# kevalmorabia97/CoVA-Web-Object-Detection

Hardware: AMD Instinct MI355X
Metric: webpages/sec fwd+bwd (90 bboxes, K=24) (higher is better)
Workload: dtype f32

## Files before the change

### cova-web-object-detection_amd/csrc/conv_wino4.hip

```cpp
#include "common.h"
#include "mma.h"
#include "bn_tail.h"
#include "options.h"
#include <type_traits>

#ifndef W4_ABL
#define W4_ABL 0
#endif

#ifdef W4_TRACE
__device__ unsigned long long g_w4_trace[2 * 20 * 8];
#define W4_STAMP(row, slot)                                                                                  \
    do {                                                                                                     \
        const int r__ = (row);                                                                               \
        if (blockIdx.x == 0 && (wave == 0 || wave == 4) && r__ >= 0 && r__ < 20 && lane == 0)                \
            g_w4_trace[((wave >> 2) * 20 + r__) * 8 + (slot)] = __builtin_amdgcn_s_memtime();                \
    } while (0)
#else
#define W4_STAMP(row, slot) do { } while (0)
#endif

namespace {

namespace w4 {
constexpr int TH = 8, TW = 32, PH = TH + 2, PW = TW + 2, NPIX = PH * PW;
constexpr int THREADS = 512;
constexpr int SLOT_FLOATS = NPIX * 16;
constexpr int TMP_CI = 16 * 36 + 4;
constexpr int TMP_FLOATS = 8 * TMP_CI;
constexpr int VROW = 36;
constexpr int V_FLOATS = 8 * 16 * VROW;
constexpr int U_FLOATS = 8 * 8 * 9 * 64 * 4;
constexpr int U_SPLIT_DWORDS = 2 * 8 * 18 * 3 * 256;
constexpr int U_TOTAL = U_FLOATS + 2 * U_SPLIT_DWORDS;
}

// ... 4 lines not shown
    o[0] = fmaf(4.f, d[0], fmaf(-5.f, d[2], d[4]));
    o[1] = a + b;
    o[2] = a - b;
    o[3] = c + e;
    o[4] = c - e;
    o[5] = fmaf(4.f, d[1], fmaf(-5.f, d[3], d[5]));
}

__device__ __forceinline__ void at6(const float (&m)[6], float (&o)[4])
{
    const float s1 = m[1] + m[2], d1 = m[1] - m[2], s2 = m[3] + m[4], d2 = m[3] - m[4];
    o[0] = m[0] + s1 + s2;
    o[1] = fmaf(2.f, d2, d1);
    o[2] = fmaf(4.f, s2, s1);
    o[3] = fmaf(8.f, d2, d1) + m[5];
}

struct W4Epi {
    const float *addend, *act, *z, *mean, *invstd, *msc, *msh;
    const uint32_t *act_bits;
    int inf_relu;
    int inference;
};

struct W4Args {
    const float *in, *in2, *u;
    float *out, *stat_part;
    int H, W, tiles_x, tiles_y, ntiles;
    const float *pro_abc;
    int pro_relu;
    W4Epi epi;
    BnTail tail;
};

__device__ __attribute__((aligned(256))) float g_w4_zero_page[64];

__device__ __forceinline__ float quad_class_sum(float v)
{
    v += __builtin_bit_cast(float, __builtin_amdgcn_update_dpp(0, __builtin_bit_cast(int, v), 0x124, 0xF, 0xF, true));
    v += __builtin_bit_cast(float, __builtin_amdgcn_update_dpp(0, __builtin_bit_cast(int, v), 0x128, 0xF, 0xF, true));
    v += __shfl_xor(v, 16, 64);
    v += __shfl_xor(v, 32, 64);
    return v;
}

template <bool STATS, int PRO, bool ADD, int BN>
__global__ __launch_bounds__(w4::THREADS, 1) void conv3x3_c64_wino4_kernel(const W4Args a)
{
    using namespace w4;
    typedef const W4Args __attribute__((address_space(4))) *KArgs;
    auto late_args = [&]() -> KArgs {
        unsigned long long kp = (unsigned long long)__builtin_amdgcn_kernarg_segment_ptr();
        asm volatile("" : "+s"(kp));
        return (KArgs)kp;
    };
    constexpr int NSLOT = 2;
    constexpr int NT = PRO == 2 ? 2 : 1;
    constexpr int IN_FLOATS = NSLOT * SLOT_FLOATS;
    __shared__ __attribute__((aligned(16))) float lds[NT * IN_FLOATS + 2 * TMP_FLOATS + 2 * V_FLOATS];
    __shared__ __attribute__((aligned(16))) float s_epi[BN ? 256 : 4];
    __shared__ float s_pro[PRO ? 192 : 1];
    __shared__ __attribute__((aligned(16))) float s_red[STATS ? 8 * 32 : 4];
    float *s_in = lds;
    float *s_in2 = lds + IN_FLOATS;
    float *s_tmp1 = lds + NT * IN_FLOATS;
    float *s_tmp0 = s_tmp1 + TMP_FLOATS;
// ... 271 lines not shown
        mfma_range(8, 12);
        item_finish(1, it, s2);
        item_read(2, it, slot2, coff2, tmp_w, tmp_r, v_w);
        mfma_range(12, 16);
        read_v(1);
        item_finish(2, it, s2);
        mfma_range(16, 36);
        } else {
        Item it0, it1, it2;
        item_read(0, it0, slot2, coff2, tmp_w, tmp_r, v_w);
        item_read(1, it1, slot2, coff2, tmp_w, tmp_r, v_w);
        item_read(2, it2, slot2, coff2, tmp_w, tmp_r, v_w);
        read_v(0);
        W4_STAMP(g - 32, 1);
        mfma_range(0, 16);
        W4_STAMP(g - 32, 2);
        read_v(1);
        mfma_range(16, 18);
        item_finish(0, it0, s2);
        item_finish(1, it1, s2);
        item_finish(2, it2, s2);
        W4_STAMP(g - 32, 3);
        mfma_range(18, 36);
        }
        W4_STAMP(g - 32, 4);
        wait_planes(g);
        W4_STAMP(g - 32, 5);
        lds_barrier();
        W4_STAMP(g - 32, 6);
    };

    constexpr bool W4_SIGNED_TILES = false;
    constexpr bool w4_neg = false;
#include "conv_wino4_epi.h"

#pragma unroll 1
    for (int g = 0; g < G; g += 2) {
        iteration(g, std::integral_constant<int, 0>{}, Ea);
        iteration(g + 1, std::integral_constant<int, 1>{}, Ea);
        if ((g & 7) == 6) tile_epilogue(g >> 3);
    }
#include "conv_wino4_tail.h"
}

struct PrepW { const float *w[4]; };
__device__ void prep_wino4s_element(const float *__restrict__ w, uint16_t *__restrict__ u_fwd, uint16_t *__restrict__ u_dgrad, int idx);
__global__ void prep_wino4_kernel(const PrepW pw, float *__restrict__ u_fwd, float *__restrict__ u_dgrad)
{
    const int idx = blockIdx.x * blockDim.x + threadIdx.x;
    if (idx >= w4::U_FLOATS) return;
    const float *__restrict__ w = pw.w[blockIdx.y];
    u_fwd += (size_t)blockIdx.y * w4::U_TOTAL;
    u_dgrad += (size_t)blockIdx.y * w4::U_TOTAL;
    const int e = idx & 3, lane = (idx >> 2) & 63, rest = idx >> 8;
    const int q = rest % 9, ws = rest / 9, wv = ws & 7, s = ws >> 3;
    const int n = 4 * q + e, kg = n / 18, p = n - 18 * kg;
    const int cog = wv & 3, ph = wv >> 2, kq = lane >> 4, l15 = lane & 15;
    const int o = cog * 16 + l15, c = 8 * s + 4 * kg + kq;
    const int il = p / 6, j = p % 6;
    const int i = ph == 0 ? il : (il == 0 ? 5 : 2 + il);
    const float G[6][3] = {{0.25f, 0.f, 0.f},
                           {-1.f / 6, -1.f / 6, -1.f / 6},
                           {-1.f / 6, 1.f / 6, -1.f / 6},
                           {1.f / 24, 1.f / 12, 1.f / 6},
                           {1.f / 24, -1.f / 12, 1.f / 6},
                           {0.f, 0.f, 1.f}};
    double uf = 0.0, ud = 0.0;
#pragma unroll
    for (int r = 0; r < 3; ++r)
#pragma unroll
        for (int t = 0; t < 3; ++t) {
            const double coef = (double)G[i][r] * (double)G[j][t];
            uf += coef * (double)w[((o * 64 + c) * 3 + r) * 3 + t];
// ... 5 lines not shown
}

#include "conv_wino4_split.h"

}

#ifdef W4_TRACE
COVA_API int cova_w4_trace_read(unsigned long long *host)
{
    return (int)hipMemcpyFromSymbol(host, HIP_SYMBOL(g_w4_trace), sizeof(unsigned long long) * 320);
}
#endif

COVA_API int cova_conv3x3_wino4_num_tiles(int B, int H, int W)
{
    return B * cdiv(W, w4::TW) * cdiv(H, w4::TH);
}

static int w4_grid(int B, int H, int W)
{
    const int tiles_x = cdiv(W, w4::TW), tiles_y = cdiv(H, w4::TH);
    int g = cova_internal_persistent_grid2(B * tiles_x * tiles_y, 1);
    const int len_odd = B * tiles_x * (tiles_y / 2);
    if (len_odd > 0) {
        if (g > 2 * len_odd) g = 2 * len_odd;
        g &= ~1;
        if (g < 2) g = 2;
    }
    return g;
}

COVA_API int cova_conv3x3_wino4_num_partials(int B, int H, int W) { return w4_grid(B, H, W); }

COVA_API int cova_conv3x3_wino4_u_floats(void) { return w4::U_TOTAL; }

COVA_API int cova_conv3x3_wino4_prep_multi(const float *w0, const float *w1, const float *w2, const float *w3,
                                           float *u_fwd, float *u_dgrad, void *stream)
{
    COVA_REQUIRE(w0 && u_fwd && u_dgrad);
    const PrepW pw{{w0, w1, w2, w3}};
    const int n = w1 == nullptr ? 1 : w2 == nullptr ? 2 : w3 == nullptr ? 3 : 4;
    hipLaunchKernelGGL(prep_wino4_kernel, dim3(cdiv(w4::U_FLOATS, 256), n), dim3(256), 0, (hipStream_t)stream, pw, u_fwd,
                       u_dgrad);
    COVA_LAUNCH_CHECK();
    return COVA_OK;
}

COVA_API int cova_conv3x3_wino4_prep(const float *w_oihw, float *u_fwd, float *u_dgrad, void *stream)
{
    return cova_conv3x3_wino4_prep_multi(w_oihw, nullptr, nullptr, nullptr, u_fwd, u_dgrad, stream);
}

namespace {

template <bool STATS, int PRO, bool ADD, int BN>
void launch_w4(const W4Args &a, int grid, hipStream_t st)
{
    if constexpr (PRO != 2) {
        if (!cova_options().wino4_f32) {
            W4Args b = a;
            b.u = a.u + w4::U_FLOATS;
            hipLaunchKernelGGL((conv3x3_c64_wino4s_kernel<STATS, PRO, ADD, BN>), dim3(grid), dim3(w4::THREADS), 0, st, b);
            return;
        }
    }
    hipLaunchKernelGGL((conv3x3_c64_wino4_kernel<STATS, PRO, ADD, BN>), dim3(grid), dim3(w4::THREADS), 0, st, a);
// ... 93 lines not shown
```

### cova-web-object-detection_amd/csrc/conv_wino4_epi.h

```cpp
    float *xw = s_x + (cog * 8 * 64 + lane) * 4;
    auto tile_epilogue = [&](int k) {
        int ph_e = ph;
        asm volatile("" : "+s"(ph_e));
        const float cf_s = ph_e == 0 ? 1.f : 4.f, cf_t0 = ph_e == 0 ? 1.f : 0.f;
        const float cf_d = ph_e == 0 ? 1.f : 8.f, cf_t1 = ph_e == 0 ? 0.f : 1.f, cf_h = ph_e == 0 ? 1.f : 2.f;
        if (W4_ABL & 32) {
#pragma unroll
            for (int p = 0; p < 18; ++p) { asm volatile("" ::"v"(acc[p])); acc[p] = f32x4{0.f, 0.f, 0.f, 0.f}; }
            return;
        }
        const int tile_ = tile_of(k);
        const int tx = tile_ % a.tiles_x, ty = (tile_ / a.tiles_x) % a.tiles_y, b = tile_ / (a.tiles_x * a.tiles_y);
        const float tsign = (W4_SIGNED_TILES && w4_neg) ? -1.f : 1.f;
        const KArgs la = late_args();
        const float *e_addend = la->epi.addend, *e_z = la->epi.z, *e_act = la->epi.act;
        float *e_out = la->out;
        float yo[2][4][4], ys[2][4][4];
#pragma unroll
        for (int r = 0; r < 4; ++r) {
            float tm[3][4];
#pragma unroll
            for (int il = 0; il < 3; ++il) {
                float m[6], o[4];
#pragma unroll
                for (int j = 0; j < 6; ++j) m[j] = acc[il * 6 + j][r];
                at6(m, o);
#pragma unroll
                for (int j = 0; j < 4; ++j) tm[il][j] = o[j];
            }
#pragma unroll
            for (int j = 0; j < 4; ++j) {
                const float sm = tm[1][j] + tm[2][j], df = tm[1][j] - tm[2][j];
                yo[0][j][r] = fmaf(cf_s, sm, cf_t0 * tm[0][j]);
                yo[1][j][r] = fmaf(cf_d, df, cf_t1 * tm[0][j]);
                ys[0][j][r] = sm;
                ys[1][j][r] = cf_h * df;
            }
        }
        const int t2 = lane >> 2, cq = cog * 16 + (lane & 3) * 4;
        const int oy0 = ty * TH + 4 * (t2 >> 3) + 2 * ph, ox0 = tx * TW + 4 * (t2 & 7);
        const size_t img = (size_t)b * H * W * 64;
        struct Ops { float4 ad[4], z4[4], a4[4]; };
        const bool bits = BN == 2 && la->epi.act_bits != nullptr;
        auto offs = [&](int io, int j) {
            return (unsigned)((min(oy0 + io, H - 1) * W + min(ox0 + j, W - 1)) * 64 + cq);
        };
        auto load_ops = [&](int io, Ops &o) {
#pragma unroll
            for (int j = 0; j < 4; ++j) {
                const unsigned off = offs(io, j);
                o.ad[j] = o.z4[j] = o.a4[j] = make_float4(0.f, 0.f, 0.f, 0.f);
                if (ADD) o.ad[j] = *reinterpret_cast<const float4 *>(e_addend + img + off);
                if (BN == 1 || BN == 2) o.z4[j] = *reinterpret_cast<const float4 *>(e_z + img + off);
                if (BN == 2) {
                    if (bits) {
                        const uint32_t wd = la->epi.act_bits[((size_t)b * H * W * 64 + off) >> 5] >> (cq & 31);
                        o.a4[j] = make_float4((float)(wd & 1u), (float)((wd >> 1) & 1u), (float)((wd >> 2) & 1u),
                                              (float)((wd >> 3) & 1u));
                    } else {
                        o.a4[j] = *reinterpret_cast<const float4 *>(e_act + img + off);
                    }
                }
            }
        };
        Ops ops;
        W4_STAMP(16 + 2 * (k - 4), 0);
        if (ADD || BN) load_ops(0, ops);
        float4 rx[2][4];
        auto put = [&]() {
#pragma unroll
            for (int io = 0; io < 2; ++io)
#pragma unroll
                for (int j = 0; j < 4; ++j)
                    *reinterpret_cast<float4 *>(xw + (io * 4 + j) * 256) = make_float4(ys[io][j][0], ys[io][j][1], ys[io][j][2], ys[io][j][3]);
        };
        auto get = [&]() {
#pragma unroll
            for (int io = 0; io < 2; ++io)
#pragma unroll
                for (int j = 0; j < 4; ++j) rx[io][j] = *reinterpret_cast<const float4 *>(xw + (io * 4 + j) * 256);
        };
        W4_STAMP(16 + 2 * (k - 4), 1);
        if (ph == 1) put();
        if (!(W4_ABL & 512)) lds_barrier();
        if (ph == 0) { get(); put(); }
        if (!(W4_ABL & 512)) lds_barrier();
        if (ph == 1) get();
        if (!(W4_ABL & 512)) lds_barrier();
        W4_STAMP(16 + 2 * (k - 4), 2);
// ... 8 lines not shown
        float ssum[4] = {0.f, 0.f, 0.f, 0.f}, ssq[4] = {0.f, 0.f, 0.f, 0.f};
#pragma unroll
        for (int io = 0; io < 2; ++io) {
            const int oy = oy0 + io;
            float mu[4] = {0.f, 0.f, 0.f, 0.f}, is[4] = {0.f, 0.f, 0.f, 0.f}, msc[4] = {0.f, 0.f, 0.f, 0.f}, msh[4] = {0.f, 0.f, 0.f, 0.f};
            if (BN) {
                const float4 m4 = *reinterpret_cast<const float4 *>(s_epi + cq), i4 = *reinterpret_cast<const float4 *>(s_epi + 64 + cq);
                mu[0] = m4.x; mu[1] = m4.y; mu[2] = m4.z; mu[3] = m4.w;
                is[0] = i4.x; is[1] = i4.y; is[2] = i4.z; is[3] = i4.w;
                if (BN == 1 || BN == 3) {
                    const float4 s4 = *reinterpret_cast<const float4 *>(s_epi + 128 + cq), h4 = *reinterpret_cast<const float4 *>(s_epi + 192 + cq);
                    msc[0] = s4.x; msc[1] = s4.y; msc[2] = s4.z; msc[3] = s4.w;
                    msh[0] = h4.x; msh[1] = h4.y; msh[2] = h4.z; msh[3] = h4.w;
                }
            }
#pragma unroll
            for (int j = 0; j < 4; ++j) {
                const bool ok = oy < H && ox0 + j < W;
                const int src = ((lane & 3) * 16 + (lane >> 2)) * 4;
                float own[4];
#pragma unroll
                for (int r = 0; r < 4; ++r)
                    own[r] = __builtin_bit_cast(float, __builtin_amdgcn_ds_bpermute(src, __builtin_bit_cast(int, yo[io][j][r])));
                const float adv[4] = {ops.ad[j].x, ops.ad[j].y, ops.ad[j].z, ops.ad[j].w};
                const float zv[4] = {ops.z4[j].x, ops.z4[j].y, ops.z4[j].z, ops.z4[j].w};
                const float av[4] = {ops.a4[j].x, ops.a4[j].y, ops.a4[j].z, ops.a4[j].w};
                float o[4];
#pragma unroll
                for (int r = 0; r < 4; ++r) {
                    float v = W4_SIGNED_TILES ? own[r] * tsign : own[r];
                    if (BN == 3) {
                        v = fmaf(msc[r], v, msh[r]);
                        if (ADD) v += adv[r];
                        if (la->epi.inf_relu) v = v > 0.f ? v : 0.f;
                        o[r] = v;
                        continue;
                    }
                    if (ADD) v += adv[r];
                    if (BN) {
                        const float gate = BN == 2 ? av[r] : fmaf(msc[r], zv[r], msh[r]);
                        if (!(gate > 0.f) || !ok) v = 0.f;
                        ssum[r] += v;
                        ssq[r] += v * ((zv[r] - mu[r]) * is[r]);
                    } else if (STATS) {
                        if (!ok) v = 0.f;
                        ssum[r] += v;
                        ssq[r] += v * v;
                    }
                    o[r] = v;
                }
                if (!(W4_ABL & 256) && ok)
                    *reinterpret_cast<float4 *>(e_out + img + (unsigned)(((oy0 + io) * W + ox0 + j) * 64 + cq)) =
                        make_float4(o[0], o[1], o[2], o[3]);
            }
            if ((ADD || BN) && io == 0) {
                __builtin_amdgcn_sched_barrier(0);
                load_ops(1, ops);
            }
        }
        W4_STAMP(16 + 2 * (k - 4), 3);
        if (STATS) {
#pragma unroll
            for (int r = 0; r < 4; ++r) {
                ssum[r] = quad_class_sum(ssum[r]);
                ssq[r] = quad_class_sum(ssq[r]);
            }
            if (lane < 4) {
// ... 13 lines not shown
```

### cova-web-object-detection_amd/csrc/conv_wino4_split.h

```cpp
namespace w4s {
constexpr int SLOT_BYTES = w4::NPIX * 64 + 64;
constexpr int PLANES_BYTES = 4 * SLOT_BYTES;
constexpr int VBLK = 1024;
constexpr int VBUF_BYTES = 12 * 3 * VBLK;
constexpr int LDS_BYTES = PLANES_BYTES + 2 * VBUF_BYTES;
constexpr int U_KSTEP_BYTES = 8 * 18 * 3 * 1024;
constexpr int U_DWORDS = 2 * U_KSTEP_BYTES / 4;
}

#ifndef W4S_ABL
#define W4S_ABL 0
#endif
#ifndef W4S_LEAD
#define W4S_LEAD 3
#endif

__device__ __forceinline__ f32x4 mfma16bf(u32x4 a, u32x4 b, f32x4 c)
{
    return __builtin_amdgcn_mfma_f32_16x16x32_bf16(__builtin_bit_cast(bf16x8, a), __builtin_bit_cast(bf16x8, b), c, 0, 0, 0);
}

template <bool STATS, int PRO, bool ADD, int BN>
__global__ __launch_bounds__(w4::THREADS, 1) void conv3x3_c64_wino4s_kernel(const W4Args a)
{
    using namespace w4;
    static_assert(PRO != 2, "the two-tensor prologue runs on the f32 main loop");
    typedef const W4Args __attribute__((address_space(4))) *KArgs;
    auto late_args = [&]() -> KArgs {
        unsigned long long kp = (unsigned long long)__builtin_amdgcn_kernarg_segment_ptr();
        asm volatile("" : "+s"(kp));
        return (KArgs)kp;
    };
    __shared__ __attribute__((aligned(256))) float lds[w4s::LDS_BYTES / 4];
    __shared__ __attribute__((aligned(16))) float s_epi[BN ? 256 : 4];
    __shared__ __attribute__((aligned(16))) float s_pro[PRO ? 192 : 4];
    __shared__ __attribute__((aligned(16))) float s_red[STATS ? 8 * 32 : 4];
    char *const s_planes = reinterpret_cast<char *>(lds);
    char *const s_vb = s_planes + w4s::PLANES_BYTES;
    float *s_x = reinterpret_cast<float *>(s_vb + w4s::VBUF_BYTES);
    const int tid = threadIdx.x, lane = tid & 63;
    const int wave = __builtin_amdgcn_readfirstlane(tid >> 6);
    const int cog = wave & 3, ph = wave >> 2;
    const int l15 = lane & 15, kq = lane >> 4;
    const int H = a.H, W = a.W;
    if (PRO && tid < 192) s_pro[tid] = late_args()->pro_abc[tid];
    if (BN && tid >= 256) {
        const int c = tid & 63, kind = (tid >> 6) & 3;
        const KArgs la = late_args();
        const float *src = kind == 0 ? la->epi.mean : kind == 1 ? la->epi.invstd : kind == 2 ? la->epi.msc : la->epi.msh;
        const bool used = BN == 3 ? kind >= 2 : (kind < 2 || BN == 1);
        s_epi[kind * 64 + c] = used ? src[c] : 0.f;
    }
    if (PRO || BN) __syncthreads();

    const int Gd = (int)gridDim.x;
    const bool lists = a.tiles_y > 1;
    const int w4_par = lists ? (int)(blockIdx.x & 1) : 0;
    const int Gp = lists ? Gd >> 1 : Gd;
    int bp = lists ? (int)(blockIdx.x >> 1) : (int)blockIdx.x;
    if ((Gd & 7) == 0) bp = lists ? (int)((blockIdx.x & 7) >> 1) * (Gd >> 3) + (int)(blockIdx.x >> 3)
                                  : (int)(blockIdx.x & 7) * (Gd >> 3) + (int)(blockIdx.x >> 3);
    const int nrow = lists ? (w4_par ? a.tiles_y >> 1 : (a.tiles_y + 1) >> 1) : a.tiles_y;
    const int per_page = nrow * a.tiles_x;
    const int lenp = (a.ntiles / (a.tiles_x * a.tiles_y)) * per_page;
    const int nk = bp < lenp ? (lenp - bp + Gp - 1) / Gp : 0;
    auto tile_of = [&](int k) {
        const int m = bp + (k < nk ? k : nk - 1) * Gp;
        const int b_ = m / per_page, rem = m - b_ * per_page, j = rem / a.tiles_x, tx_ = rem - j * a.tiles_x;
        return (b_ * a.tiles_y + (lists ? 2 * j + w4_par : j)) * a.tiles_x + tx_;
    };
    const bool w4_neg = w4_par != 0;

    const unsigned pl_base = (unsigned)(size_t)(lds_void *)s_planes;
    const float *tbase = a.in;
    unsigned rel16[3] = {0, 0, 0};
    bool in16[3] = {false, false, false};
    const int q16 = lane & 3;
    auto px16 = [&](int i) { return 16 * (wave + 8 * i) + (lane >> 2); };
#pragma unroll
    for (int i = 0; i < 3; ++i) {
        const int px = px16(i), r = px / PW, c = px - r * PW;
        rel16[i] = (unsigned)((r * W + c) * 64 + 4 * q16) * 4u;
    }
    auto plane_src = [&](int k) {
        const int tile_ = tile_of(k);
        const int tx = tile_ % a.tiles_x, ty = (tile_ / a.tiles_x) % a.tiles_y, b = tile_ / (a.tiles_x * a.tiles_y);
        const long long org = ((long long)b * H * W + (long long)(ty * TH - 1) * W + (tx * TW - 1)) * 64;
        tbase = a.in + org;
#pragma unroll
        for (int i = 0; i < 3; ++i) {
            int px = px16(i);
            asm volatile("" : "+v"(px));
            const int r = (px * 241) >> 13, c = px - r * PW;
            const int gy = ty * TH + r - 1, gx = tx * TW + c - 1;
            in16[i] = gy >= 0 && gy < H && gx >= 0 && gx < W;
        }
    };
    auto copy_piece = [&](const int gi, const int slot, const int i) {
        if (W4S_ABL & 8) return;
        const int j = wave + 8 * i;
        if (j < 22 && px16(i) < NPIX) {
            const unsigned dst = pl_base + (unsigned)slot * w4s::SLOT_BYTES + j * 1024;
            if (in16[i]) copy16_to_lds(tbase + 16 * gi, rel16[i], dst);
            else copy16_to_lds(g_w4_zero_page, (unsigned)q16 * 16u, dst);
        }
    };

    const int hf = wave & 1;
    const int tt = 4 * (wave >> 1) + (lane >> 4), cp = lane & 15;
    const int tt_rd = (W4S_ABL & 512) ? (tt & ~1) : tt;
    const char *rd = s_planes + (cp >> 3) * w4s::SLOT_BYTES + ((4 * (tt_rd >> 3) + hf) * PW + 4 * (tt_rd & 7)) * 64 + (cp & 7) * 8;
    char *vw = s_vb + hf * (6 * 3 * w4s::VBLK) + tt * 64 + ((((cp >> 2) ^ ((4 - (tt >> 2)) & 3))) << 4) + (cp & 3) * 4;
    const char *vr = s_vb + ph * (6 * 3 * w4s::VBLK) + l15 * 64 + ((kq ^ ((4 - (l15 >> 2)) & 3)) << 4);
    unsigned m30 = 0x3FFFFFFFu;
    bool edge = false;
    auto masks = [&](int k) {
        const int tile_ = tile_of(k);
        const int tx_ = tile_ % a.tiles_x, ty_ = (tile_ / a.tiles_x) % a.tiles_y;
        edge = ty_ == 0 || ty_ * TH + TH + 1 > H || tx_ == 0 || tx_ * TW + TW + 1 > W;
        const int gy0 = ty_ * TH + 4 * (tt >> 3) + hf - 1, gx0 = tx_ * TW + 4 * (tt & 7) - 1;
        unsigned cm = 0, m = 0;
#pragma unroll
        for (int c = 0; c < 6; ++c) cm |= (gx0 + c >= 0 && gx0 + c < W) ? (1u << c) : 0u;
#pragma unroll
        for (int r = 0; r < 5; ++r) m |= (gy0 + r >= 0 && gy0 + r < H) ? (cm << (6 * r)) : 0u;
        m30 = m;
    };

    float T[3][6][2];
#pragma unroll
    for (int i = 0; i < 3; ++i)
#pragma unroll
        for (int c = 0; c < 6; ++c) T[i][c][0] = T[i][c][1] = 0.f;
    auto column = [&](const int c, const int par, const int ks, auto edge_t) {
        constexpr bool EDGE = decltype(edge_t)::value;
        if (W4S_ABL & 1) return;
        const char *p = rd + par * (2 * w4s::SLOT_BYTES) + c * 64;
        float x[5][2];
#pragma unroll
        for (int r = 0; r < 5; ++r) {
            const float2 v = *reinterpret_cast<const float2 *>(p + r * (PW * 64));
            x[r][0] = v.x; x[r][1] = v.y;
        }
        if (PRO) {
            const float2 A2 = *reinterpret_cast<const float2 *>(s_pro + 32 * ks + 2 * cp);
            const float2 C2 = *reinterpret_cast<const float2 *>(s_pro + 128 + 32 * ks + 2 * cp);
            const float Av[2] = {A2.x, A2.y}, Cv[2] = {C2.x, C2.y};
#pragma unroll
            for (int r = 0; r < 5; ++r)
#pragma unroll
                for (int e = 0; e < 2; ++e) {
// ... 12 lines not shown
                o1 = u + v; o2 = u - v;
            } else {
                const float u = x[3][e] - x[1][e], v = 2.f * (x[2][e] - x[0][e]);
                o1 = u + v; o2 = u - v;
            }
            T[0][c][e] = o0; T[1][c][e] = o1; T[2][c][e] = o2;
        }
    };
    auto column_e = [&](const int c, const int par, const int ks) {
        if (PRO && edge) column(c, par, ks, std::true_type{});
        else column(c, par, ks, std::false_type{});
    };
    auto row_stage = [&](const int sn, float (&o)[6][2]) {
        if (W4S_ABL & 1) return;
#pragma unroll
        for (int e = 0; e < 2; ++e) {
            const float d[6] = {T[sn][0][e], T[sn][1][e], T[sn][2][e], T[sn][3][e], T[sn][4][e], T[sn][5][e]};
            float r[6];
            bt6(d, r);
#pragma unroll
            for (int j = 0; j < 6; ++j) o[j][e] = r[j];
        }
    };
    auto split_write = [&](const int j, const int parw, const float (&o)[6][2]) {
        if (W4S_ABL & 1) return;
        uint32_t q0, q1, q2;
        bf3_split_pair(o[j][0], o[j][1], q0, q1, q2);
        char *d = vw + parw * w4s::VBUF_BYTES + j * (3 * w4s::VBLK);
        *reinterpret_cast<uint32_t *>(d) = q0;
        *reinterpret_cast<uint32_t *>(d + w4s::VBLK) = q1;
        *reinterpret_cast<uint32_t *>(d + 2 * w4s::VBLK) = q2;
    };

    const char *const ubase = reinterpret_cast<const char *>(a.u) + (size_t)wave * (18 * 3 * 1024) +
                              (w4_neg ? (size_t)w4::U_SPLIT_DWORDS * 4 : (size_t)0);
    const unsigned ulane = (unsigned)lane * 16u;
    constexpr int UR = W4S_LEAD + 1;
    static_assert(36 % UR == 0, "ring size must divide the 36-position stream");
    u32x4 Ub[UR][3];
    auto load_u = [&](const int n_, const int slot) {
        if (W4S_ABL & 16) return;
        const int n = n_ % 36;
        const char *ub_t = ubase;
        const int ks = (W4S_ABL & 128) ? 0 : n / 18, p = (W4S_ABL & 128) ? 0 : n - 18 * ks;
        if (W4S_ABL & 256) {
#pragma unroll
            for (int q = 0; q < 3; ++q) Ub[slot][q] = *reinterpret_cast<const u32x4 *>(vr + ((n % 12) * 3 + q) * w4s::VBLK);
            return;
        }
        const char *bp = ub_t + (size_t)ks * w4s::U_KSTEP_BYTES + p * 3072;
        unsigned ul = ulane;
        asm volatile("" : "+v"(ul));
#pragma unroll
        for (int q = 0; q < 3; ++q) Ub[slot][q] = *reinterpret_cast<const u32x4 *>(bp + q * 1024 + ul);
    };

    plane_src(0);
#pragma unroll
    for (int i = 0; i < 3; ++i)
#pragma unroll
        for (int g = 0; g < 4; ++g) copy_piece(g, g, i);
#pragma unroll
    for (int n = 0; n < UR; ++n)
#pragma unroll
        for (int q = 0; q < 3; ++q) Ub[n][q] = u32x4{0u, 0u, 0u, 0u};
#pragma unroll
    for (int n = 0; n < W4S_LEAD; ++n) load_u(n, n);
    __builtin_amdgcn_s_waitcnt(0);
    __syncthreads();
    if (PRO) masks(0);
    {
#pragma unroll
        for (int c = 0; c < 6; ++c) column_e(c, 0, 0);
        float o[6][2];
        row_stage(0, o);
#pragma unroll
        for (int j = 0; j < 6; ++j) split_write(j, 0, o);
    }
    if (STATS && tid < 256) s_red[tid] = 0.f;
    __syncthreads();

    f32x4 acc[18];
#pragma unroll
    for (int p = 0; p < 18; ++p) acc[p] = f32x4{0.f, 0.f, 0.f, 0.f};

    auto step = [&](const int k, auto ks_t, auto s_t) {
        constexpr int KS = decltype(ks_t)::value, S = decltype(s_t)::value;
        constexpr int TI = 3 * KS + S, PAR = TI & 1, NPAR = (KS + 1) & 1, NKS = NPAR;
        if (KS == 0 && S == 0) plane_src(k + 1);
        copy_piece(2 * KS, 2 * KS, S);
        copy_piece(2 * KS + 1, 2 * KS + 1, S);
        if (PRO && KS == 1 && S == 1) masks(k + 1);
        const char *vp = vr + PAR * w4s::VBUF_BYTES;
        u32x4 Vr[2][3];
        auto read_v = [&](const int j, const int b) {
            if (W4S_ABL & 64) return;
#pragma unroll
            for (int q = 0; q < 3; ++q) Vr[b][q] = *reinterpret_cast<const u32x4 *>(vp + (j * 3 + q) * w4s::VBLK);
        };
        float o[6][2];
        if (W4S_ABL & 64) {
#pragma unroll
            for (int q = 0; q < 3; ++q) Vr[0][q] = Vr[1][q] = u32x4{0u, 0u, 0u, 0u};
        }
        read_v(0, 0);
        if (S != 2) row_stage(S + 1, o);
#pragma unroll
        for (int j = 0; j < 6; ++j) {
            constexpr int n0 = TI * 6;
            const int n = n0 + j, ub = n % UR;
            if (j < 5) read_v(j + 1, (j + 1) & 1);
            if (!(W4S_ABL & 4)) {
                f32x4 c = acc[S * 6 + j];
                const u32x4 *U = Ub[ub], *V = Vr[j & 1];
                c = mfma16bf(U[2], V[0], c);
                c = mfma16bf(U[0], V[2], c);
                c = mfma16bf(U[1], V[1], c);
                c = mfma16bf(U[1], V[0], c);
                c = mfma16bf(U[0], V[1], c);
                c = mfma16bf(U[0], V[0], c);
                acc[S * 6 + j] = c;
            }
            load_u(n + W4S_LEAD, (n + W4S_LEAD) % UR);
            if (S == 0) {
                split_write(j, PAR ^ 1, o);
            } else if (S == 1) {
                split_write(j, PAR ^ 1, o);
                if (j >= 3) column_e(j - 3, NPAR, NKS);
            } else {
                if (j < 3) column_e(3 + j, NPAR, NKS);
                if (j == 2) row_stage(0, o);
                if (j >= 3) { split_write(2 * (j - 3), PAR ^ 1, o); split_write(2 * (j - 3) + 1, PAR ^ 1, o); }
            }
        }
        lds_barrier();
    };

    constexpr bool W4_SIGNED_TILES = true;
#include "conv_wino4_epi.h"

    using I0 = std::integral_constant<int, 0>;
    using I1 = std::integral_constant<int, 1>;
    using I2 = std::integral_constant<int, 2>;
#pragma unroll 1
    for (int k = 0; k < nk; ++k) {
        step(k, I0{}, I0{});
        step(k, I0{}, I1{});
        step(k, I0{}, I2{});
        step(k, I1{}, I0{});
        step(k, I1{}, I1{});
        step(k, I1{}, I2{});
        tile_epilogue(k);
    }
    asm volatile("s_waitcnt vmcnt(0)" ::: "memory");
#include "conv_wino4_tail.h"
}

static_assert(2 * 8 * 18 * 64 * 8 == w4::U_FLOATS, "one thread of prep_wino4_kernel per element of either image");
__device__ void prep_wino4s_element(const float *__restrict__ w, uint16_t *__restrict__ u_fwd, uint16_t *__restrict__ u_dgrad, int idx)
{
    const int e = idx & 7, lane = (idx >> 3) & 63, rest = idx >> 9;
    const int p = rest % 18, wv = (rest / 18) & 7, ks = rest / (18 * 8);
    const int cog = wv & 3, ph = wv >> 2, kq = lane >> 4, l15 = lane & 15;
    const int o = cog * 16 + l15, c = 32 * ks + 8 * kq + e;
    const int il = p / 6, j = p % 6;
    const int i = ph == 0 ? il : (il == 0 ? 5 : 2 + il);
    const float G[6][3] = {{0.25f, 0.f, 0.f},
                           {-1.f / 6, -1.f / 6, -1.f / 6},
                           {-1.f / 6, 1.f / 6, -1.f / 6},
                           {1.f / 24, 1.f / 12, 1.f / 6},
                           {1.f / 24, -1.f / 12, 1.f / 6},
                           {0.f, 0.f, 1.f}};
    double uf = 0.0, ud = 0.0;
#pragma unroll
    for (int r = 0; r < 3; ++r)
#pragma unroll
        for (int t = 0; t < 3; ++t) {
            const double coef = (double)G[i][r] * (double)G[j][t];
            uf += coef * (double)w[((o * 64 + c) * 3 + r) * 3 + t];
            ud += coef * (double)w[((c * 64 + o) * 3 + (2 - r)) * 3 + (2 - t)];
        }
    const size_t base = ((((size_t)ks * 8 + wv) * 18 + p) * 3) * 512 + lane * 8 + e;
    uint32_t q0, q1, q2;
    bf3_split_pair((float)uf, (float)ud, q0, q1, q2);
    constexpr size_t NEG = 2 * (size_t)w4::U_SPLIT_DWORDS;
// ... 11 lines not shown
```

### cova-web-object-detection_amd/csrc/mma.h

```cpp
#pragma once
#include "bf3.h"

__device__ __forceinline__ f32x4 mfma16x4(float a, float b, f32x4 c)
{
    return __builtin_amdgcn_mfma_f32_16x16x4f32(a, b, c, 0, 0, 0);
}

__device__ __forceinline__ f32x16 mfma32bf(u32x4 a, u32x4 b, f32x16 c)
{
    return __builtin_amdgcn_mfma_f32_32x32x16_bf16(__builtin_bit_cast(bf16x8, a), __builtin_bit_cast(bf16x8, b), c, 0, 0, 0);
}

typedef __attribute__((address_space(3))) void lds_void;

__device__ __forceinline__ void copy16_to_lds(const void *base, unsigned off_bytes, unsigned lds_base_bytes)
{
    asm volatile("s_mov_b32 m0, %0\n\tglobal_load_lds_dwordx4 %1, %2" ::"s"(lds_base_bytes), "v"(off_bytes), "s"(base) : "memory", "m0");
}

template <int IMM, int LDS_ADD>
__device__ __forceinline__ void copy16_to_lds_imm(const void *base, unsigned off_bytes, unsigned lds_base_bytes)
{
    static_assert(IMM >= 0 && IMM < 4096, "global_load_lds: 13-bit signed immediate offset");
    static_assert(LDS_ADD >= 0 && LDS_ADD < 65536, "LDS byte offset");
    if constexpr (LDS_ADD == 0)
        asm volatile("s_mov_b32 m0, %0\n\tglobal_load_lds_dwordx4 %1, %2 offset:%3" ::"s"(lds_base_bytes), "v"(off_bytes), "s"(base), "i"(IMM) : "memory", "m0");
    else
        asm volatile("s_add_u32 m0, %0, %4\n\tglobal_load_lds_dwordx4 %1, %2 offset:%3" ::"s"(lds_base_bytes), "v"(off_bytes), "s"(base), "i"(IMM), "i"(LDS_ADD) : "memory", "m0", "scc");
}

__device__ __forceinline__ void lds_barrier() { asm volatile("s_waitcnt lgkmcnt(0)\n\ts_barrier" ::: "memory"); }
```

### include/cova_hip.h

```cpp
#ifndef COVA_HIP_H
#define COVA_HIP_H

#include <stdint.h>

#ifdef __cplusplus
extern "C" {
#endif

#define COVA_ERR_BAD_ARG 10001

typedef struct cova_bn_tail {
    int mode;
    int *counter;
    double count;
    const float *gamma, *beta;
    float *running_mean, *running_var;
    long long *num_batches_tracked;
    float momentum, eps;
    float *scale, *shift, *mean, *invstd;
    float *dgamma, *dbeta, *abc;
} cova_bn_tail;

int cova_conv_out_size(int in_size, int kernel, int stride, int pad);
int cova_set_option(int key, int value);

int cova_conv1_prep_weights(const float *w_oihw , float *w_k , void *stream);

int cova_conv1_num_tiles(int B, int H, int W);
int cova_conv1_num_partials(int B, int H, int W);
int cova_conv1_fwd(const float *img, const float *w_k, float *out, float *stat_part, int B, int H,
                   int W, void *stream);
int cova_conv1_fwd_tail(const float *img, const float *w_oihw, float *out, float *stat_part, int B, int H, int W,
                        const cova_bn_tail *tail, void *stream);
int cova_conv1_wgrad_workspace_floats(int B, int H, int W);
int cova_conv1_wgrad(const float *img, const float *dy , float *dw, float *ws, int B, int H,
                     int W, void *stream);
int cova_pool_bwd_dy1(const float *dp, const uint8_t *idx, const float *y1, const float *abc, float *dy1, int B, int H1,
                      int W1, void *stream);
int cova_conv1_dgrad(const float *dy1, const float *w_oihw, float *dimg, int B, int H, int W, void *stream);
int cova_conv1_wgrad_poolbwd(const float *img, const float *y1, const float *dp, const uint8_t *idx,
                             const float *abc, float *dw, float *ws, int B, int H, int W,
                             void *stream);

int cova_conv3x3_wgrad4_num_partials(int B, int H, int W);
int cova_conv3x3_wgrad4_workspace_floats(int B, int H, int W);
int cova_conv3x3_wgrad4_partial(const float *act, const float *act_abc , int act_relu, const float *dz,
                                const float *dz2 , const float *dz_abc ,
                                float *dz_out , float *ws, int B,
                                int H, int W, void *stream);
int cova_conv3x3_wgrad4_finish(const float *ws0, float *dw0, const float *ws1, float *dw1, const float *ws2,
                               float *dw2, const float *ws3, float *dw3, int B, int H, int W, void *stream);
int cova_conv3x3_wgrad4(const float *act, const float *dz, float *dw , float *ws, int B, int H, int W,
                        void *stream);

int cova_conv3x3_wino4_u_floats(void);
int cova_conv3x3_wino4_num_tiles(int B, int H, int W);
int cova_conv3x3_wino4_num_partials(int B, int H, int W);
int cova_conv3x3_wino4_prep(const float *w_oihw, float *u_fwd, float *u_dgrad, void *stream);
int cova_conv3x3_wino4_prep_multi(const float *w0, const float *w1, const float *w2, const float *w3, float *u_fwd,
                                  float *u_dgrad, void *stream);
int cova_conv3x3_wino4(const float *in, const float *u, float *out, float *stat_part , int B, int H,
                       int W, void *stream);
int cova_conv3x3_wino4_pro(const float *in, const float *pro_abc, int pro_relu, const float *u, float *out,
                           float *stat_part , int B, int H, int W, void *stream);
int cova_conv3x3_wino4_full(const float *in, const float *in2 , const float *pro_abc ,
                            int pro_relu, const float *u, const float *addend ,
                            const float *act , const float *mask_scale ,
                            const float *mask_shift , const float *z ,
                            const float *mean , const float *invstd , float *out,
                            float *stat_part , int B, int H, int W, void *stream);
int cova_conv3x3_wino4_full_tail(const float *in, const float *in2 , const float *pro_abc ,
                                 int pro_relu, const float *u, const float *addend ,
                                 const float *act , const uint32_t *act_bits ,
                                 const float *mask_scale ,
                                 const float *mask_shift , const float *z ,
                                 const float *mean , const float *invstd , float *out,
                                 float *stat_part, int B, int H, int W, const cova_bn_tail *tail, void *stream);
int cova_conv3x3_wino4_bnact(const float *in, const float *pro_abc , int pro_relu, const float *u,
                             const float *addend , const float *scale, const float *shift, int relu,
                             float *out, int B, int H, int W, void *stream);

int cova_conv1x1_num_partials(long long R, int Cin, int Cout);
int cova_conv1x1(const float *in, const float *in2 , const float *pro_abc ,
                 int pro_relu, const float *w, int w_trans, const float *addend ,
                 const float *act , const uint32_t *act_bits ,
                 const float *mask_scale ,
                 const float *mask_shift , const float *z ,
                 const float *mean , const float *invstd ,
                 const float *z2 , const float *mean2 ,
                 const float *invstd2 , float *out, float *stat_part ,
// ... 305 lines not shown
```

Baseline: 1826.

## Walk tiles incrementally and hoist epilogue pointers and copy addressing in split Winograd kernel

```diff
diff --git a/cova-web-object-detection_amd/csrc/conv_wino4.hip b/cova-web-object-detection_amd/csrc/conv_wino4.hip
--- a/cova-web-object-detection_amd/csrc/conv_wino4.hip
+++ b/cova-web-object-detection_amd/csrc/conv_wino4.hip
@@ -2,6 +2,7 @@
 #include "mma.h"
 #include "bn_tail.h"
 #include "options.h"
+#include "conv_wino4_walk.h"
 #include <type_traits>
 
 #ifndef W4_ABL
@@ -72,6 +73,25 @@
     W4Epi epi;
     BnTail tail;
 };
+
+struct W4EpiOps {
+    const float *addend, *z, *act;
+    const uint32_t *act_bits;
+    float *out;
+    int inf_relu;
+};
+template <bool ADD, int BN, class KA>
+__device__ __forceinline__ W4EpiOps w4_epi_ops(KA la)
+{
+    W4EpiOps o;
+    o.addend = ADD ? la->epi.addend : nullptr;
+    o.z = (BN == 1 || BN == 2) ? la->epi.z : nullptr;
+    o.act = BN == 2 ? la->epi.act : nullptr;
+    o.act_bits = BN == 2 ? la->epi.act_bits : nullptr;
+    o.out = la->out;
+    o.inf_relu = BN == 3 ? la->epi.inf_relu : 0;
+    return o;
+}
 
 __device__ __attribute__((aligned(256))) float g_w4_zero_page[64];
 
@@ -409,13 +429,17 @@
 
     constexpr bool W4_SIGNED_TILES = false;
     constexpr bool w4_neg = false;
+    auto epi_ops = [&]() { return w4_epi_ops<ADD, BN>(late_args()); };
 #include "conv_wino4_epi.h"
 
 #pragma unroll 1
     for (int g = 0; g < G; g += 2) {
         iteration(g, std::integral_constant<int, 0>{}, Ea);
         iteration(g + 1, std::integral_constant<int, 1>{}, Ea);
-        if ((g & 7) == 6) tile_epilogue(g >> 3);
+        if ((g & 7) == 6) {
+            const int tile_ = tile_of(g >> 3);
+            tile_epilogue(g >> 3, tile_ % a.tiles_x, (tile_ / a.tiles_x) % a.tiles_y, tile_ / (a.tiles_x * a.tiles_y));
+        }
     }
 #include "conv_wino4_tail.h"
 }
@@ -487,6 +511,23 @@
 
 COVA_API int cova_conv3x3_wino4_num_partials(int B, int H, int W) { return w4_grid(B, H, W); }
 
+COVA_API int cova_conv3x3_wino4_walk_tiles(int B, int H, int W, int grid, int stride, int *tiles, int *counts)
+{
+    if (!(tiles && counts && B > 0 && H > 0 && W > 0 && grid >= 0 && stride > 0)) return -1;
+    const int tiles_x = cdiv(W, w4::TW), tiles_y = cdiv(H, w4::TH), ntiles = B * tiles_x * tiles_y;
+    if (grid == 0) grid = w4_grid(B, H, W);
+    for (int block = 0; block < grid; ++block) {
+        w4walk::Walk wk = w4walk::walk_init(block, grid, tiles_x, tiles_y, ntiles);
+        if (wk.nk + 1 > stride) return -1;
+        counts[block] = wk.nk;
+        for (int k = 0; k <= wk.nk; ++k) {
+            tiles[(size_t)block * stride + k] = (wk.b * tiles_y + w4walk::walk_ty(wk)) * tiles_x + wk.tx;
+            w4walk::walk_next(wk, k + 1, tiles_x);
+        }
+    }
+    return grid;
+}
+
 COVA_API int cova_conv3x3_wino4_u_floats(void) { return w4::U_TOTAL; }
 
 COVA_API int cova_conv3x3_wino4_prep_multi(const float *w0, const float *w1, const float *w2, const float *w3,
diff --git a/cova-web-object-detection_amd/csrc/conv_wino4_epi.h b/cova-web-object-detection_amd/csrc/conv_wino4_epi.h
--- a/cova-web-object-detection_amd/csrc/conv_wino4_epi.h
+++ b/cova-web-object-detection_amd/csrc/conv_wino4_epi.h
@@ -1,5 +1,5 @@
     float *xw = s_x + (cog * 8 * 64 + lane) * 4;
-    auto tile_epilogue = [&](int k) {
+    auto tile_epilogue = [&](int k, const int tx, const int ty, const int b) {
         int ph_e = ph;
         asm volatile("" : "+s"(ph_e));
         const float cf_s = ph_e == 0 ? 1.f : 4.f, cf_t0 = ph_e == 0 ? 1.f : 0.f;
@@ -9,12 +9,10 @@
             for (int p = 0; p < 18; ++p) { asm volatile("" ::"v"(acc[p])); acc[p] = f32x4{0.f, 0.f, 0.f, 0.f}; }
             return;
         }
-        const int tile_ = tile_of(k);
-        const int tx = tile_ % a.tiles_x, ty = (tile_ / a.tiles_x) % a.tiles_y, b = tile_ / (a.tiles_x * a.tiles_y);
         const float tsign = (W4_SIGNED_TILES && w4_neg) ? -1.f : 1.f;
-        const KArgs la = late_args();
-        const float *e_addend = la->epi.addend, *e_z = la->epi.z, *e_act = la->epi.act;
-        float *e_out = la->out;
+        const W4EpiOps eo = epi_ops();
+        const float *e_addend = eo.addend, *e_z = eo.z, *e_act = eo.act;
+        float *e_out = eo.out;
         float yo[2][4][4], ys[2][4][4];
 #pragma unroll
         for (int r = 0; r < 4; ++r) {
@@ -41,7 +39,7 @@
         const int oy0 = ty * TH + 4 * (t2 >> 3) + 2 * ph, ox0 = tx * TW + 4 * (t2 & 7);
         const size_t img = (size_t)b * H * W * 64;
         struct Ops { float4 ad[4], z4[4], a4[4]; };
-        const bool bits = BN == 2 && la->epi.act_bits != nullptr;
+        const bool bits = BN == 2 && eo.act_bits != nullptr;
         auto offs = [&](int io, int j) {
             return (unsigned)((min(oy0 + io, H - 1) * W + min(ox0 + j, W - 1)) * 64 + cq);
         };
@@ -54,7 +52,7 @@
                 if (BN == 1 || BN == 2) o.z4[j] = *reinterpret_cast<const float4 *>(e_z + img + off);
                 if (BN == 2) {
                     if (bits) {
-                        const uint32_t wd = la->epi.act_bits[((size_t)b * H * W * 64 + off) >> 5] >> (cq & 31);
+                        const uint32_t wd = eo.act_bits[((size_t)b * H * W * 64 + off) >> 5] >> (cq & 31);
                         o.a4[j] = make_float4((float)(wd & 1u), (float)((wd >> 1) & 1u), (float)((wd >> 2) & 1u),
                                               (float)((wd >> 3) & 1u));
                     } else {
@@ -129,7 +127,7 @@
                     if (BN == 3) {
                         v = fmaf(msc[r], v, msh[r]);
                         if (ADD) v += adv[r];
-                        if (la->epi.inf_relu) v = v > 0.f ? v : 0.f;
+                        if (eo.inf_relu) v = v > 0.f ? v : 0.f;
                         o[r] = v;
                         continue;
                     }
diff --git a/cova-web-object-detection_amd/csrc/conv_wino4_split.h b/cova-web-object-detection_amd/csrc/conv_wino4_split.h
--- a/cova-web-object-detection_amd/csrc/conv_wino4_split.h
+++ b/cova-web-object-detection_amd/csrc/conv_wino4_split.h
@@ -53,28 +53,17 @@
     }
     if (PRO || BN) __syncthreads();
 
-    const int Gd = (int)gridDim.x;
-    const bool lists = a.tiles_y > 1;
-    const int w4_par = lists ? (int)(blockIdx.x & 1) : 0;
-    const int Gp = lists ? Gd >> 1 : Gd;
-    int bp = lists ? (int)(blockIdx.x >> 1) : (int)blockIdx.x;
-    if ((Gd & 7) == 0) bp = lists ? (int)((blockIdx.x & 7) >> 1) * (Gd >> 3) + (int)(blockIdx.x >> 3)
-                                  : (int)(blockIdx.x & 7) * (Gd >> 3) + (int)(blockIdx.x >> 3);
-    const int nrow = lists ? (w4_par ? a.tiles_y >> 1 : (a.tiles_y + 1) >> 1) : a.tiles_y;
-    const int per_page = nrow * a.tiles_x;
-    const int lenp = (a.ntiles / (a.tiles_x * a.tiles_y)) * per_page;
-    const int nk = bp < lenp ? (lenp - bp + Gp - 1) / Gp : 0;
-    auto tile_of = [&](int k) {
-        const int m = bp + (k < nk ? k : nk - 1) * Gp;
-        const int b_ = m / per_page, rem = m - b_ * per_page, j = rem / a.tiles_x, tx_ = rem - j * a.tiles_x;
-        return (b_ * a.tiles_y + (lists ? 2 * j + w4_par : j)) * a.tiles_x + tx_;
-    };
-    const bool w4_neg = w4_par != 0;
+    w4walk::Walk wk = w4walk::walk_init((int)blockIdx.x, (int)gridDim.x, a.tiles_x, a.tiles_y, a.ntiles);
+    const int nk = wk.nk;
+    const int tiles_x = a.tiles_x;
+    const bool w4_neg = wk.par != 0;
+    int c_tx = 0, c_ty = 0, c_b = 0;
 
     const unsigned pl_base = (unsigned)(size_t)(lds_void *)s_planes;
+    const unsigned pl_wave = pl_base + (unsigned)wave * 1024u;
     const float *tbase = a.in;
     unsigned rel16[3] = {0, 0, 0};
-    bool in16[3] = {false, false, false};
+    bool in16[3] = {false, false, false}, out16_2 = false;
     const int q16 = lane & 3;
     auto px16 = [&](int i) { return 16 * (wave + 8 * i) + (lane >> 2); };
 #pragma unroll
@@ -82,28 +71,31 @@
         const int px = px16(i), r = px / PW, c = px - r * PW;
         rel16[i] = (unsigned)((r * W + c) * 64 + 4 * q16) * 4u;
     }
-    auto plane_src = [&](int k) {
-        const int tile_ = tile_of(k);
-        const int tx = tile_ % a.tiles_x, ty = (tile_ / a.tiles_x) % a.tiles_y, b = tile_ / (a.tiles_x * a.tiles_y);
-        const long long org = ((long long)b * H * W + (long long)(ty * TH - 1) * W + (tx * TW - 1)) * 64;
-        tbase = a.in + org;
+    const int HW = H * W;
+    const int px_end2 = wave + 16 < 22 ? NPIX : 0;
+    auto plane_src = [&]() {
+        const int tx = wk.tx, ty = w4walk::walk_ty(wk), b = wk.b;
+        tbase = a.in + (long long)b * HW * 64 + ((ty * TH - 1) * W + (tx * TW - 1)) * 64;
 #pragma unroll
         for (int i = 0; i < 3; ++i) {
             int px = px16(i);
             asm volatile("" : "+v"(px));
             const int r = (px * 241) >> 13, c = px - r * PW;
             const int gy = ty * TH + r - 1, gx = tx * TW + c - 1;
-            in16[i] = gy >= 0 && gy < H && gx >= 0 && gx < W;
-        }
-    };
-    auto copy_piece = [&](const int gi, const int slot, const int i) {
+            const bool inside = gy >= 0 && gy < H && gx >= 0 && gx < W;
+            const bool there = i < 2 || px < px_end2;
+            in16[i] = there && inside;
+            if (i == 2) out16_2 = there && !inside;
+        }
+    };
+    const float *zpage = g_w4_zero_page;
+    asm volatile("" : "+s"(zpage));
+    auto copy_piece = [&](auto slot_t, auto i_t) {
+        constexpr int SL = decltype(slot_t)::value, I = decltype(i_t)::value;
+        constexpr int DST = SL * w4s::SLOT_BYTES + I * 8192;
         if (W4S_ABL & 8) return;
-        const int j = wave + 8 * i;
-        if (j < 22 && px16(i) < NPIX) {
-            const unsigned dst = pl_base + (unsigned)slot * w4s::SLOT_BYTES + j * 1024;
-            if (in16[i]) copy16_to_lds(tbase + 16 * gi, rel16[i], dst);
-            else copy16_to_lds(g_w4_zero_page, (unsigned)q16 * 16u, dst);
-        }
+        if (in16[I]) copy16_to_lds_imm<64 * SL, DST - 64 * SL>(tbase, rel16[I], pl_wave);
+        else if (I < 2 || out16_2) copy16_to_lds_imm<0, DST>(zpage, (unsigned)q16 * 16u, pl_wave);
     };
 
     const int hf = wave & 1;
@@ -114,9 +106,8 @@
     const char *vr = s_vb + ph * (6 * 3 * w4s::VBLK) + l15 * 64 + ((kq ^ ((4 - (l15 >> 2)) & 3)) << 4);
     unsigned m30 = 0x3FFFFFFFu;
     bool edge = false;
-    auto masks = [&](int k) {
-        const int tile_ = tile_of(k);
-        const int tx_ = tile_ % a.tiles_x, ty_ = (tile_ / a.tiles_x) % a.tiles_y;
+    auto masks = [&]() {
+        const int tx_ = wk.tx, ty_ = w4walk::walk_ty(wk);
         edge = ty_ == 0 || ty_ * TH + TH + 1 > H || tx_ == 0 || tx_ * TW + TW + 1 > W;
         const int gy0 = ty_ * TH + 4 * (tt >> 3) + hf - 1, gx0 = tx_ * TW + 4 * (tt & 7) - 1;
         unsigned cm = 0, m = 0;
@@ -195,8 +186,10 @@
         *reinterpret_cast<uint32_t *>(d + 2 * w4s::VBLK) = q2;
     };
 
-    const char *const ubase = reinterpret_cast<const char *>(a.u) + (size_t)wave * (18 * 3 * 1024) +
-                              (w4_neg ? (size_t)w4::U_SPLIT_DWORDS * 4 : (size_t)0);
+    typedef const u32x4 __attribute__((address_space(1))) *UPtr;
+    typedef const char __attribute__((address_space(1))) *UBytes;
+    unsigned long long up = (unsigned long long)(reinterpret_cast<const char *>(a.u) + (size_t)wave * (18 * 3 * 1024) +
+                                                 (w4_neg ? (size_t)w4::U_SPLIT_DWORDS * 4 : (size_t)0));
     const unsigned ulane = (unsigned)lane * 16u;
     constexpr int UR = W4S_LEAD + 1;
     static_assert(36 % UR == 0, "ring size must divide the 36-position stream");
@@ -204,25 +197,31 @@
     auto load_u = [&](const int n_, const int slot) {
         if (W4S_ABL & 16) return;
         const int n = n_ % 36;
-        const char *ub_t = ubase;
-        const int ks = (W4S_ABL & 128) ? 0 : n / 18, p = (W4S_ABL & 128) ? 0 : n - 18 * ks;
         if (W4S_ABL & 256) {
 #pragma unroll
             for (int q = 0; q < 3; ++q) Ub[slot][q] = *reinterpret_cast<const u32x4 *>(vr + ((n % 12) * 3 + q) * w4s::VBLK);
             return;
         }
-        const char *bp = ub_t + (size_t)ks * w4s::U_KSTEP_BYTES + p * 3072;
-        unsigned ul = ulane;
-        asm volatile("" : "+v"(ul));
-#pragma unroll
-        for (int q = 0; q < 3; ++q) Ub[slot][q] = *reinterpret_cast<const u32x4 *>(bp + q * 1024 + ul);
-    };
-
-    plane_src(0);
-#pragma unroll
-    for (int i = 0; i < 3; ++i)
-#pragma unroll
-        for (int g = 0; g < 4; ++g) copy_piece(g, g, i);
+#pragma unroll
+        for (int q = 0; q < 3; ++q) Ub[slot][q] = *reinterpret_cast<UPtr>(reinterpret_cast<UBytes>(up) + ulane + q * 1024);
+        if (W4S_ABL & 128) return;
+        up += n == 17 ? (unsigned long long)(w4s::U_KSTEP_BYTES - 17 * 3072)
+                      : n == 35 ? 0ull - (unsigned long long)(w4s::U_KSTEP_BYTES + 17 * 3072) : 3072ull;
+        asm volatile("" : "+s"(up));
+    };
+
+    plane_src();
+    {
+        auto prime_row = [&](auto i_t) {
+            copy_piece(std::integral_constant<int, 0>{}, i_t);
+            copy_piece(std::integral_constant<int, 1>{}, i_t);
+            copy_piece(std::integral_constant<int, 2>{}, i_t);
+            copy_piece(std::integral_constant<int, 3>{}, i_t);
+        };
+        prime_row(std::integral_constant<int, 0>{});
+        prime_row(std::integral_constant<int, 1>{});
+        prime_row(std::integral_constant<int, 2>{});
+    }
 #pragma unroll
     for (int n = 0; n < UR; ++n)
 #pragma unroll
@@ -231,7 +230,7 @@
     for (int n = 0; n < W4S_LEAD; ++n) load_u(n, n);
     __builtin_amdgcn_s_waitcnt(0);
     __syncthreads();
-    if (PRO) masks(0);
+    if (PRO) masks();
     {
 #pragma unroll
         for (int c = 0; c < 6; ++c) column_e(c, 0, 0);
@@ -250,10 +249,14 @@
     auto step = [&](const int k, auto ks_t, auto s_t) {
         constexpr int KS = decltype(ks_t)::value, S = decltype(s_t)::value;
         constexpr int TI = 3 * KS + S, PAR = TI & 1, NPAR = (KS + 1) & 1, NKS = NPAR;
-        if (KS == 0 && S == 0) plane_src(k + 1);
-        copy_piece(2 * KS, 2 * KS, S);
-        copy_piece(2 * KS + 1, 2 * KS + 1, S);
-        if (PRO && KS == 1 && S == 1) masks(k + 1);
+        if (KS == 0 && S == 0) {
+            c_tx = wk.tx; c_ty = w4walk::walk_ty(wk); c_b = wk.b;
+            w4walk::walk_next(wk, k + 1, tiles_x);
+            plane_src();
+        }
+        copy_piece(std::integral_constant<int, 2 * KS>{}, s_t);
+        copy_piece(std::integral_constant<int, 2 * KS + 1>{}, s_t);
+        if (PRO && KS == 1 && S == 1) masks();
         const char *vp = vr + PAR * w4s::VBUF_BYTES;
         u32x4 Vr[2][3];
         auto read_v = [&](const int j, const int b) {
@@ -300,6 +303,12 @@
     };
 
     constexpr bool W4_SIGNED_TILES = true;
+    constexpr bool EPI_HELD = PRO == 0;
+    const W4EpiOps epi_held = w4_epi_ops<ADD, BN>(late_args());
+    auto epi_ops = [&]() {
+        if constexpr (EPI_HELD) return epi_held;
+        else return w4_epi_ops<ADD, BN>(late_args());
+    };
 #include "conv_wino4_epi.h"
 
     using I0 = std::integral_constant<int, 0>;
@@ -313,7 +322,7 @@
         step(k, I1{}, I0{});
         step(k, I1{}, I1{});
         step(k, I1{}, I2{});
-        tile_epilogue(k);
+        tile_epilogue(k, c_tx, c_ty, c_b);
     }
     asm volatile("s_waitcnt vmcnt(0)" ::: "memory");
 #include "conv_wino4_tail.h"
diff --git a/cova-web-object-detection_amd/csrc/conv_wino4_walk.h b/cova-web-object-detection_amd/csrc/conv_wino4_walk.h
--- /dev/null
+++ b/cova-web-object-detection_amd/csrc/conv_wino4_walk.h
@@ -0,0 +1,49 @@
+#pragma once
+
+namespace w4walk {
+
+struct Walk {
+    int par;
+    int nk;
+    int nrow, ymul;
+    int b, j, tx;
+    int db, dj, dtx;
+};
+
+__host__ __device__ inline Walk walk_init(int block, int Gd, int tiles_x, int tiles_y, int ntiles)
+{
+    const bool lists = tiles_y > 1;
+    Walk w;
+    w.par = lists ? (block & 1) : 0;
+    w.ymul = lists ? 2 : 1;
+    const int Gp = lists ? Gd >> 1 : Gd;
+    int bp = lists ? block >> 1 : block;
+    if ((Gd & 7) == 0) bp = lists ? ((block & 7) >> 1) * (Gd >> 3) + (block >> 3) : (block & 7) * (Gd >> 3) + (block >> 3);
+    w.nrow = lists ? (w.par ? tiles_y >> 1 : (tiles_y + 1) >> 1) : tiles_y;
+    const int per_page = w.nrow * tiles_x;
+    const int lenp = (ntiles / (tiles_x * tiles_y)) * per_page;
+    w.nk = bp < lenp ? (lenp - bp + Gp - 1) / Gp : 0;
+    if (w.nk == 0) bp = 0;
+    w.b = bp / per_page;
+    int r = bp - w.b * per_page;
+    w.j = r / tiles_x;
+    w.tx = r - w.j * tiles_x;
+    w.db = Gp / per_page;
+    r = Gp - w.db * per_page;
+    w.dj = r / tiles_x;
+    w.dtx = r - w.dj * tiles_x;
+    return w;
+}
+
+__host__ __device__ inline void walk_next(Walk &w, int k_next, int tiles_x)
+{
+    if (k_next >= w.nk) return;
+    int tx = w.tx + w.dtx, j = w.j + w.dj, b = w.b + w.db;
+    if (tx >= tiles_x) { tx -= tiles_x; ++j; }
+    if (j >= w.nrow) { j -= w.nrow; ++b; }
+    w.tx = tx; w.j = j; w.b = b;
+}
+
+__host__ __device__ inline int walk_ty(const Walk &w) { return w.ymul * w.j + w.par; }
+
+}
diff --git a/cova-web-object-detection_amd/csrc/mma.h b/cova-web-object-detection_amd/csrc/mma.h
--- a/cova-web-object-detection_amd/csrc/mma.h
+++ b/cova-web-object-detection_amd/csrc/mma.h
@@ -22,7 +22,7 @@
 __device__ __forceinline__ void copy16_to_lds_imm(const void *base, unsigned off_bytes, unsigned lds_base_bytes)
 {
     static_assert(IMM >= 0 && IMM < 4096, "global_load_lds: 13-bit signed immediate offset");
-    static_assert(LDS_ADD >= 0 && LDS_ADD < 65536, "LDS byte offset");
+    static_assert(LDS_ADD >= 0 && LDS_ADD < 160 * 1024, "LDS byte offset (a 32-bit literal of the scalar add)");
     if constexpr (LDS_ADD == 0)
         asm volatile("s_mov_b32 m0, %0\n\tglobal_load_lds_dwordx4 %1, %2 offset:%3" ::"s"(lds_base_bytes), "v"(off_bytes), "s"(base), "i"(IMM) : "memory", "m0");
     else
diff --git a/include/cova_hip.h b/include/cova_hip.h
--- a/include/cova_hip.h
+++ b/include/cova_hip.h
@@ -56,6 +56,7 @@
 int cova_conv3x3_wino4_u_floats(void);
 int cova_conv3x3_wino4_num_tiles(int B, int H, int W);
 int cova_conv3x3_wino4_num_partials(int B, int H, int W);
+int cova_conv3x3_wino4_walk_tiles(int B, int H, int W, int grid, int stride, int *tiles, int *counts);
 int cova_conv3x3_wino4_prep(const float *w_oihw, float *u_fwd, float *u_dgrad, void *stream);
 int cova_conv3x3_wino4_prep_multi(const float *w0, const float *w1, const float *w2, const float *w3, float *u_fwd,
                                   float *u_dgrad, void *stream);
```

New measurement: 1824. No clear change (-0.1%).
